# jacky121298/3DAL_PyTorch

Hardware: AMD Instinct MI355X
Metric: object-crops/sec through static+dynamic refinement heads (higher is better)
Workload: dtype f32; 1 GPU; StaticModelOneBoxEst forward+decode, 4096 crops x 1024 pts per GPU, fp32 (BASELINE.json configs[1]); items_per_gpu=4096, points_per_item=1024, sampler=device, parallelism=single GPU

## Files before the change

### 3dal_pytorch_amd/_hip.py

```python
import ctypes as C
import os

import numpy as np
import torch

_HERE = os.path.dirname(os.path.abspath(__file__))
LIB_PATH = os.path.join(_HERE, "lib3dal_hip.so")

OK, EINVAL, EWORKSPACE, EHIP = 0, -1, -2, -3
F32, BF16, F16, F16X3 = 0, 1, 2, 3
DTYPES = {"fp32": F32, "bf16": BF16, "fp16": F16, "f16x3": F16X3}
HEAD_INS_SEG, HEAD_STATIC_BOX_EST, HEAD_POINT_EMB, HEAD_BOX_EMB, HEAD_DYNAMIC_BOX_EST = range(5)
SAMPLER_DEVICE, SAMPLER_CHOICE = 0, 1
PHASE_SEG, PHASE_BOX, PHASE_ALL = 1, 2, 3

vp = C.c_void_p


class Layer(C.Structure):
    _fields_ = [("weight", vp), ("bias", vp), ("bn_weight", vp), ("bn_bias", vp), ("bn_mean", vp),
                ("bn_var", vp), ("c_in", C.c_int32), ("c_out", C.c_int32)]


class PackItem(C.Structure):
# ... 315 lines not shown
class AugmentBoxesArgs(C.Structure):
    _fields_ = [("B", C.c_int64), ("max_gt", C.c_int32), ("max_cand", C.c_int32), ("max_objs", C.c_int32), ("n_classes", C.c_int32),
                ("transform", C.c_int32), ("reserved", C.c_int32), ("gt_boxes", vp), ("gt_classes", vp), ("gt_counts", vp),
                ("cand_boxes", vp), ("cand_classes", vp), ("cand_counts", vp), ("accept", vp), ("xform", vp),
                ("range", C.c_float * 4), ("out", vp), ("out_count", vp), ("status", vp)]


_i, _i64, _u64, _sz = C.c_int, C.c_int64, C.c_uint64, C.c_size_t
SIGNATURES = {
    "dal3_version": (_i, []),
    "dal3_last_error": (C.c_char_p, []),
    "dal3_mean_size": (C.POINTER(C.c_float), []),
    "dal3_pack_weights": (_i, [_i, C.POINTER(Layer), _i, _i, vp, C.POINTER(_sz), vp]),
    "dal3_ins_seg_workspace_bytes": (_sz, [_i]),
    "dal3_ins_seg_plan_layout": (_i, [_i, C.POINTER(_sz), C.POINTER(_i)]),
    "dal3_ins_seg_forward": (_i, [vp, _i, _i, BCN, _i, _i, vp, vp, vp, vp, _sz, vp]),
    "dal3_ins_seg_encode": (_i, [vp, _i, _i, BCN, _i, _i, vp, vp]),
    "dal3_ins_seg_global_bias": (_i, [vp, _i, vp, _i, vp, vp]),
    "dal3_ins_seg_decode": (_i, [vp, _i, _i, BCN, _i, _i, vp, vp, vp, vp]),
    "dal3_gather_workspace_bytes": (_sz, [_i, _i]),
    "dal3_segment_counts": (_i, [vp, _i, _i, vp, vp]),
    "dal3_mask_compact_sample": (_i, [vp, BCN, _i, _i, _i, _i, _i, vp, _u64, _i64, vp, vp, vp, vp, _sz, vp]),
    "dal3_mask_compact_sample_step": (_i, [vp, BCN, _i, _i, _i, _i, _u64, vp, _i64, vp, vp, vp, vp, _sz, vp]),
    "dal3_point_head_workspace_bytes": (_sz, [_i]),
    "dal3_point_head_forward": (_i, [_i, vp, _i, BCN, _i, _i, vp, _i64, vp, _sz, vp]),
    "dal3_point_head_pool_workspace_bytes": (_sz, [_i, _i]),
    "dal3_point_head_screen_min_tiles": (_i, []),
    "dal3_point_head_screen_stride": (_i, []),
    "dal3_point_head_pool": (_i, [_i, vp, _i, BCN, _i, _i, vp, vp, vp, _sz, vp]),
    "dal3_dynamic_box_est_forward": (_i, [vp, vp, _i, vp, vp, _sz, vp]),
# ... 197 lines not shown
        if offsets.is_cuda:
            raise TypeError(f"{name} must be on the host (a list, an array or a CPU tensor): {sized_by} from it, and "
                            "reading a device tensor back would be the synchronisation this call avoids")
        offsets = offsets.numpy()
    off = np.ascontiguousarray(np.asarray(offsets, dtype=np.int64).reshape(-1))
    if off.size < 1:
        raise ValueError(f"{name} needs {count} + 1 entries")
    if off[0] < 0 or off[-1] > n or np.any(np.diff(off) < 0):
        raise ValueError(f"{name} must be non-decreasing within [0, {n}]")
    return off


STORAGE = {torch.float32: F32, torch.bfloat16: BF16, torch.float16: F16}
BCN_NO_SMALL_JOB_KERNELS, BCN_NO_WORKLIST, BCN_NO_LDS_SAMPLER = 1, 2, 4
BCN_NO_DEC_PLAN = 16
DISPATCH_FLAGS = 0


def bcn(t):
    assert t.dim() == 3 and t.dtype in STORAGE
    sb, sc, sn = t.stride()
    return BCN(ptr(t), sb, sc, sn, STORAGE[t.dtype], DISPATCH_FLAGS)


def layer_struct(conv, bn):
    w = conv.weight
    c_in, c_out = getattr(conv, "in_channels", w.shape[1]), getattr(conv, "out_channels", w.shape[0])
    if not w.is_contiguous() or w.dtype != torch.float32:
        raise RuntimeError("weights must be contiguous fp32")
    L = Layer(ptr(w), ptr(conv.bias), None, None, None, None, c_in, c_out)
# ... 45 lines not shown
```

### 3dal_pytorch_amd/csrc/dal3_api.hip

```cpp
#include <stdarg.h>
#include <stdio.h>
#include <string.h>

#include "dal3_block.h"
#include "dal3_kernels.h"
#include "dal3_lp.h"

static thread_local char g_err[512] = "";

static int fail(int code, const char* fmt, ...) {
    va_list ap;
    va_start(ap, fmt);
    vsnprintf(g_err, sizeof(g_err), fmt, ap);
    va_end(ap);
    return code;
}

#define HIP_TRY(expr)                                                                           \
    do {                                                                                        \
        hipError_t e_ = (expr);                                                                 \
        if (e_ != hipSuccess) return fail(DAL3_EHIP, "%s: %s", #expr, hipGetErrorString(e_)); \
    } while (0)
#define TRY(expr)               \
    do {                        \
// ... 456 lines not shown
        HIP_TRY(launch_pack_weight(L[3], PACK_ROWMAJOR, 0, 256, 0, 0, mut(w.w4row), s));
        HIP_TRY(launch_pack_weight_lp(L[3], DAL3_F16, 0, 0, 256, 16, 8, reinterpret_cast<uint16_t*>(mut(w.w4h)), s));
        HIP_TRY(launch_pack_head_screen(L[3], mut(w.scr_pq), reinterpret_cast<int32_t*>(mut(w.scr_flag)), s));
    }
    return pack_fc(L + 4, w.fc, s);
}

static BCN to_bcn(const dal3_bcn& t) { return BCN{t.data, t.stride_b, t.stride_c, t.stride_n, t.dtype, t.flags}; }

static int check_bcn(const dal3_bcn& t, const char* what) {
    if (!t.data) return fail(DAL3_EINVAL, "%s: null data pointer", what);
    if (t.stride_n <= 0 || t.stride_c <= 0) return fail(DAL3_EINVAL, "%s: strides must be positive", what);
    if (t.dtype != DAL3_F32 && t.dtype != DAL3_BF16 && t.dtype != DAL3_F16)
        return fail(DAL3_EINVAL, "%s: storage dtype %d is none of DAL3_F32 / DAL3_BF16 / DAL3_F16", what, t.dtype);
    if (t.dtype != DAL3_F32 && (reinterpret_cast<uintptr_t>(t.data) & 1)) return fail(DAL3_EINVAL, "%s: 16-bit data must be 2-byte aligned", what);
    if (t.flags & ~(DAL3_BCN_NO_SMALL_JOB_KERNELS | DAL3_BCN_NO_WORKLIST | DAL3_BCN_NO_LDS_SAMPLER | DAL3_BCN_NO_DEC_PLAN)) return fail(DAL3_EINVAL, "%s: unknown bits in flags (%d)", what, t.flags);
    return 0;
}

static int check_extent(int64_t B, int64_t N, const char* what) {
    if (B <= 0 || N <= 0) return fail(DAL3_EINVAL, "%s: B and N must be positive (B=%lld N=%lld)", what, (long long)B, (long long)N);
    if (B > DAL3_MAX_ITEMS) return fail(DAL3_EINVAL, "%s: B=%lld items exceed DAL3_MAX_ITEMS (%d)", what, (long long)B, DAL3_MAX_ITEMS);
    if (N > DAL3_MAX_POINTS_PER_ITEM)
        return fail(DAL3_EINVAL, "%s: N=%lld points per item exceed DAL3_MAX_POINTS_PER_ITEM (%d)", what, (long long)N, DAL3_MAX_POINTS_PER_ITEM);
    if (B * ((N + 31) / 32) > (int64_t)DAL3_MAX_TILES)
        return fail(DAL3_EINVAL, "%s: B=%lld x N=%lld is %lld 32-point tiles, more than DAL3_MAX_TILES (%d): split the batch", what,
                    (long long)B, (long long)N, (long long)(B * ((N + 31) / 32)), DAL3_MAX_TILES);
    return 0;
}

struct InsSegWs { float* g; float* gb; uint32_t* prune; uint32_t* plan_k; float* plan_gbc; int32_t* plan_nch; };
// ... 10 lines not shown
extern "C" size_t dal3_ins_seg_workspace_bytes(int B) {
    Carver c(nullptr, 0);
    carve_ins_seg(c, B);
    return c.off;
}

extern "C" int dal3_ins_seg_plan_layout(int B, size_t off[4], int* min_dead) {
    if (B <= 0 || !off) return fail(DAL3_EINVAL, "ins_seg_plan_layout: bad argument");
    char* const origin = reinterpret_cast<char*>(uintptr_t(4096));
    Carver c(origin, ~size_t(0));
    const InsSegWs w = carve_ins_seg(c, B);
    off[0] = reinterpret_cast<char*>(w.prune) - origin, off[1] = reinterpret_cast<char*>(w.plan_k) - origin;
    off[2] = reinterpret_cast<char*>(w.plan_gbc) - origin, off[3] = reinterpret_cast<char*>(w.plan_nch) - origin;
    if (min_dead) *min_dead = DAL3_DEC_MIN_DEAD;
    return 0;
}

static int check_dtype(int dtype) {
    if (dtype != DAL3_F32 && dtype != DAL3_BF16 && dtype != DAL3_F16 && dtype != DAL3_F16X3)
        return fail(DAL3_EINVAL, "unknown dtype %d", dtype);
    return 0;
}

static int ins_seg_run(const void* packed, int dtype, int c_in, const dal3_bcn& pts, int B, int N, float* logits,
                       uint8_t* mask, float* global_feat_out, const InsSegWs& ws, hipStream_t s) {
    TRY(check_dtype(dtype));
    if (!packed || !logits || !mask) return fail(DAL3_EINVAL, "ins_seg: null pointer");
    TRY(check_extent(B, N, "ins_seg"));
    if (c_in != 3 && c_in != 4) return fail(DAL3_EINVAL, "ins_seg: c_in must be 3 or 4");
    TRY(check_bcn(pts, "pts"));
// ... 2079 lines not shown
```

### 3dal_pytorch_amd/csrc/dal3_enc_screen.hip

```cpp
#include "dal3_device.h"
#include "dal3_kernels.h"
#include "dal3_lp.h"
#include "dal3_screen.h"

#ifndef SCR_CAP
#define SCR_CAP 1024
#endif
#define SCR_XLD 132
#define SCR_STAGE_LD 36
#ifndef SCR_DEPTH
#define SCR_DEPTH 2
#endif
#define SCR_XMAX_BITS 0x476A6000
#ifndef DAL3_SCR_A_STRIDE
#define DAL3_SCR_A_STRIDE 4
#endif
static_assert(DAL3_SCR_A_STRIDE >= 1, "pass A's stride over the wave-slots");

#ifdef DAL3_SCREEN_COUNT
__device__ unsigned long long g_scr_count[8];
extern "C" int dal3_debug_screen_counts(unsigned long long* out, int reset) {
    hipError_t e = hipMemcpyFromSymbol(out, HIP_SYMBOL(g_scr_count), sizeof(g_scr_count));
    if (e == hipSuccess && reset) {
        unsigned long long z[8] = {};
// ... 57 lines not shown
    for (int mt = 0; mt < 16; ++mt) {
#pragma unroll
        for (int j = 0; j < T; ++j) acc[mt & 1][j] = f32x16{};
#pragma unroll
        for (int i = 0; i < 4; ++i) {
            const f16x8_t a = __builtin_bit_cast(f16x8_t, r16.slot[i]);
            r16.slot[i] = r16.fetch();
#pragma unroll
            for (int j = 0; j < T; ++j) acc[mt & 1][j] = FP16::mfma(xh[j][i >> 1].k[i & 1], a, acc[mt & 1][j]);
        }
        if (mt > 0) fold(acc[(mt - 1) & 1], mt - 1);
    }
    fold(acc[1], 15);
}

template <int PASS, int T>
__global__ __launch_bounds__(64 * DAL3_WG_WAVES) void ins_seg_encode_screen_kernel(InsSegW w, BCN pts, int c_in, int n_pts,
                                                                                  int tiles_per_item, float* __restrict__ g,
                                                                                  uint32_t* __restrict__ prune) {
    const int lane = threadIdx.x & 63;
    const int wave = threadIdx.x >> 6;
    const int h = lane >> 5;
    const int64_t b = blockIdx.x / tiles_per_item;
    const int n0 = ((blockIdx.x % tiles_per_item) * DAL3_WG_WAVES + wave) * (PASS == 0 ? DAL3_SCR_A_STRIDE : 1) * (32 * T);
    __shared__ float s_b5[1024];
    __shared__ int s_max[1024];
    __shared__ f32x2 s_pq[1024];
    __shared__ float s_g[PASS == 1 ? 1024 : 1];
    __shared__ __attribute__((aligned(16))) float s_x[PASS == 1 ? DAL3_WG_WAVES * 32 * SCR_XLD : 4];
    __shared__ uint32_t s_list[PASS == 1 ? DAL3_WG_WAVES * T * SCR_CAP : 1];
    __shared__ __attribute__((aligned(16))) uint32_t s_stage[PASS == 1 ? DAL3_WG_WAVES * 64 * SCR_STAGE_LD : 4];
    __shared__ uint32_t s_u[PASS == 1 ? 512 : 1];
    __shared__ int s_xn[1];
    int* gi = reinterpret_cast<int*>(g + b * 1024);
    static_assert(22 * 1024 + 64 + DAL3_WG_WAVES * (32 * SCR_XLD * 4 + T * SCR_CAP * 4 + 64 * SCR_STAGE_LD * 4) <= 160 * 1024,
                  "pass B's LDS exceeds a CU's 160 KiB: lower SCR_CAP, DAL3_WG_WAVES or DAL3_ENC_T");
    static_assert(32 * 64 <= 64 * SCR_STAGE_LD, "a wave's stage holds the hit words of conv5's 32 blocks");
    if (PASS == 0 && *w.scr_flag != 0) return;
    for (int i = threadIdx.x; i < 1024; i += 64 * DAL3_WG_WAVES) {
        s_b5[i] = w.b5[i];
        s_max[i] = 0;
        s_pq[i] = reinterpret_cast<const f32x2*>(w.scr_pq)[i];
        if (PASS == 1) s_g[i] = __int_as_float(__hip_atomic_load(gi + i, __ATOMIC_RELAXED, __HIP_MEMORY_SCOPE_AGENT));
        if (PASS == 1 && i < 512) s_u[i] = 0;
    }
    if (threadIdx.x == 0) s_xn[0] = 0;
    __syncthreads();
    if (n0 < n_pts) {
        WRing<DAL3_PF> ring;
        ring.init(w.enc_stream, lane);
        f32x16 bias = tile_from_channels(w.b2, h);
        float in[T][2];
        load_points<2, T>(pts, b, n0, n_pts, c_in, in, lane);
        f32x16 x1[T][2], x2[T][2], x3[T][2], x4[T][4];
        first_layer<2, 2, T>(w.w1, w.b1, in, x1, lane);
        mlp_layer_ring<2, 2, T>(ring, w.b2, w.b3, bias, x1, x2, lane);
        if (PASS == 1 && prune) dec_prune_sweep<T>(w, x2, s_u, s_xn, lane);
        mlp_layer_ring<2, 2, T>(ring, w.b3, w.b4, bias, x2, x3, lane);
        mlp_layer_ring<2, 4, T>(ring, w.b4, w.b4, bias, x3, x4, lane);
        SCR_COUNT(0, 1);

        int xm = 0;
#pragma unroll
        for (int j = 0; j < T; ++j) {
#pragma unroll
            for (int kt = 0; kt < 4; ++kt) {
#pragma unroll
                for (int r = 0; r < 16; ++r) {
                    const int v = __float_as_int(x4[j][kt][r]);
                    xm = v > xm ? v : xm;
                }
            }
        }
        const bool dense = *w.scr_flag != 0 || __builtin_amdgcn_ballot_w64(xm > SCR_XMAX_BITS) != 0;
        if (dense) {
            SCR_COUNT(1, 1);
            if (PASS == 1) conv_max_layer<4, T>(ring, s_b5, x4, reinterpret_cast<float*>(s_max), 32, lane);
        } else {
            float x2max = 0.0f;
#pragma unroll
            for (int j = 0; j < T; ++j) {
                float ss = 0.0f;
#pragma unroll
                for (int kt = 0; kt < 4; ++kt) {
#pragma unroll
                    for (int r = 0; r < 16; ++r) ss = fmaf(x4[j][kt][r], x4[j][kt][r], ss);
                }
                ss += __shfl_xor(ss, 32);
                x2max = __builtin_fmaxf(x2max, ss);
            }
#pragma unroll
            for (int d = 16; d >= 1; d >>= 1) x2max = __builtin_fmaxf(x2max, __shfl_xor(x2max, d));
            const float X = sqrtf(x2max) * (1.0f + 0x1p-16f);

            ActTile<FP16> xh[T][4];
#pragma unroll
            for (int j = 0; j < T; ++j) {
#pragma unroll
                for (int kt = 0; kt < 4; ++kt) xh[j][kt] = pack_relu<FP16>(x4[j][kt]);
            }

            uint32_t* const list = s_list + (PASS == 1 ? wave * T * SCR_CAP : 0);
            uint32_t* const stage = s_stage + (PASS == 1 ? wave * 64 * SCR_STAGE_LD : 0);
            ScreenHits<T> hits;
            hits.init();

            auto block_const = [&](int mt) -> float {
                const int c = 32 * mt + (lane & 31);
                const f32x2 pq = s_pq[c];
                float E = fmaf(X, pq[0], pq[1]);
                E = fmaf(E, 0x1p-20f, E);
                if (PASS == 0) return E;
                const float G = s_g[c], bb = s_b5[c];
                if (bits_nonfinite(G)) return 3.0e38f;
                return (G - bb) - fmaf(__builtin_fabsf(G) + __builtin_fabsf(bb), 0x1p-22f, E);
            };
            static_assert(16 * T <= 32, "one hit bit per (tile, register) in a 32-bit word");
            float m = 0.0f;
            uint32_t hb = 0;
            auto ep_slice = [&](const f32x16 (&acc)[T], int i, float k) {
#pragma unroll
                for (int rr = 0; rr < 2; ++rr) {
#pragma unroll
                    for (int j = 0; j < T; ++j) {
                        const int r = 2 * i + rr;
                        if (PASS == 0)
                            m = (r == 0 && j == 0) ? acc[0][0] : __builtin_fmaxf(m, acc[j][r]);
                        else
                            hb = scr_push_hit(hb, acc[j][r], k);
                    }
                }
            };
            auto ep_finish = [&](int mt, float k) {
                const int c = 32 * mt + (lane & 31);
                if (PASS == 0) {
                    m = __builtin_fmaxf(m, __shfl_xor(m, 32));
                    const float y = m - fmaf(__builtin_fabsf(m), 0x1p-22f, k);
                    int bits = __float_as_int(y + s_b5[c]);
                    bits = bits > 0 ? bits : 0;
                    if (lane < 32 && bits > 0) atomicMax(&s_max[c], bits);
                } else {
                    hits.park_block(stage, mt, hb, lane);
                }
            };

            WRing<8> r16;
            r16.init(w.w5h, lane);
            auto mm = [&](f32x16 (&acc)[T], auto side) {
#pragma unroll
                for (int j = 0; j < T; ++j) acc[j] = f32x16{};
#pragma unroll
                for (int i = 0; i < 8; ++i) {
                    const f16x8_t a = __builtin_bit_cast(f16x8_t, r16.slot[i]);
                    r16.slot[i] = r16.fetch();
#pragma unroll
                    for (int j = 0; j < T; ++j) acc[j] = FP16::mfma(xh[j][i >> 1].k[i & 1], a, acc[j]);
                    DAL3_SCHED_FENCE();
                    side(i);
                    DAL3_SCHED_FENCE();
                }
            };
            f32x16 accA[T], accB[T];
            float kA = block_const(0), kB;
            mm(accA, NoSide());
            int mt = 1;
            for (; mt + 1 < 32; mt += 2) {
                kB = block_const(mt);
                mm(accB, [&](int i) { ep_slice(accA, i, kA); });
                ep_finish(mt - 1, kA);
                kA = block_const(mt + 1);
                mm(accA, [&](int i) { ep_slice(accB, i, kB); });
                ep_finish(mt, kB);
            }
            kB = block_const(mt);
            mm(accB, [&](int i) { ep_slice(accA, i, kA); });
            ep_finish(mt - 1, kA);
#pragma unroll
            for (int i = 0; i < 8; ++i) ep_slice(accB, i, kB);
            ep_finish(mt, kB);

            if (PASS == 1) {
                uint32_t cnt[T];
                const bool overflow = scr_build_lists<T, 32, SCR_CAP>(stage, list, hits, cnt, lane);
#pragma unroll
                for (int j = 0; j < T; ++j) SCR_COUNT(3, cnt[j]);
                if (overflow) {
                    SCR_COUNT(2, 1);
                    WRing<DAL3_PF> r32;
                    r32.init(w.enc_stream + ENC_W5 * 64, lane);
                    conv_max_layer<4, T>(r32, s_b5, x4, reinterpret_cast<float*>(s_max), 32, lane);
                } else {
                    float* const xw = s_x + wave * 32 * SCR_XLD;
#pragma unroll
                    for (int j = 0; j < T; ++j) {
                        __builtin_amdgcn_wave_barrier();
#pragma unroll
                        for (int kt = 0; kt < 4; ++kt) {
#pragma unroll
                            for (int q = 0; q < 4; ++q) {
                                f32x4 v;
                                v[0] = x4[j][kt][4 * q + 0];
                                v[1] = x4[j][kt][4 * q + 1];
                                v[2] = x4[j][kt][4 * q + 2];
                                v[3] = x4[j][kt][4 * q + 3];
                                *reinterpret_cast<f32x4*>(xw + (lane & 31) * SCR_XLD + 32 * kt + 8 * q + 4 * h) = v;
                            }
                        }
                        __builtin_amdgcn_wave_barrier();
                        SCR_COUNT(4, (cnt[j] + 63) / 64);
                        scr_recompute<32, 4, SCR_DEPTH, true>(
                            w.w5row, 128, list + j * SCR_CAP, cnt[j], xw, SCR_XLD, stage, lane, [](uint32_t, bool) { return 0.0f; },
                            [&](float a, int c, uint32_t, bool live) {
                                int bits = __float_as_int(a + s_b5[c]);
                                bits = bits > 0 ? bits : 0;
                                if (live && bits > 0) atomicMax(&s_max[c], bits);
                            });
                    }
                }
            }
        }
    }
    __syncthreads();
    for (int c = threadIdx.x; c < 1024; c += 64 * DAL3_WG_WAVES) {
        const int v = s_max[c];
        if (v > 0) atomicMax(gi + c, v);
    }
    if (PASS == 1 && prune) {
        uint32_t* pu = prune + b * 513;
        for (int c = threadIdx.x; c < 512; c += 64 * DAL3_WG_WAVES) {
            const uint32_t v = s_u[c];
            if (v > 0) atomicMax(pu + c, v);
        }
        if (threadIdx.x == 0 && s_xn[0] > 0) atomicMax(reinterpret_cast<int*>(pu + 512), s_xn[0]);
    }
}

hipError_t launch_ins_seg_encode_screen(const InsSegW& w, BCN pts, int c_in, int B, int N, float* g, hipStream_t s, uint32_t* prune) {
    constexpr int T = DAL3_ENC_T;
    const int tpi = (N + 32 * DAL3_WG_WAVES * T - 1) / (32 * DAL3_WG_WAVES * T);
    const int slots = (N + 32 * T - 1) / (32 * T);
    const int tpi_a = ((slots + DAL3_SCR_A_STRIDE - 1) / DAL3_SCR_A_STRIDE + DAL3_WG_WAVES - 1) / DAL3_WG_WAVES;
    const dim3 grid_a((unsigned)((int64_t)B * tpi_a)), grid((unsigned)((int64_t)B * tpi)), block(64 * DAL3_WG_WAVES);
    hipLaunchKernelGGL((ins_seg_encode_screen_kernel<0, T>), grid_a, block, 0, s, w, pts, c_in, N, tpi_a, g, nullptr);
    hipError_t e = hipGetLastError();
    if (e != hipSuccess) return e;
    hipLaunchKernelGGL((ins_seg_encode_screen_kernel<1, T>), grid, block, 0, s, w, pts, c_in, N, tpi, g, prune);
    return hipGetLastError();
}
```

### 3dal_pytorch_amd/csrc/dal3_kernels.h

```cpp
#pragma once
#include <hip/hip_runtime.h>
#include <stddef.h>
#include <stdint.h>

#include "../../include/dal3.h"
#include "dal3_device.h"
#include "dal3_fold.h"

#ifndef DAL3_ENC_T
#define DAL3_ENC_T 2
#endif
#ifndef DAL3_DEC_T
#define DAL3_DEC_T 1
#endif
#ifndef DAL3_HEAD_T
#define DAL3_HEAD_T 1
#endif

#ifndef DAL3_ENC_SCREEN
#define DAL3_ENC_SCREEN 1
#endif

#ifndef DAL3_WG_WAVES
#define DAL3_WG_WAVES 4
// ... 159 lines not shown
hipError_t launch_pack_weight_lp(const dal3_layer& L, int dtype, int kt_major, int col_off, int n_cols, int mt_n, int kt_n,
                                 uint16_t* out, hipStream_t s, int grp_blocks = 0, int64_t grp_a0 = 0, int64_t grp_a1 = 0,
                                 int64_t grp_stride = 0);

size_t ins_seg_packed_floats(int c_in);
InsSegW ins_seg_view(const float* base, int c_in);
size_t point_head_packed_floats(int head_kind);
PointHeadW point_head_view(const float* base, int head_kind);
size_t fc_head_packed_floats();
FcW fc_head_view(const float* base);
void point_head_dims(int head_kind, int* c_in, int* ks, int c[4], int* n_fc, int fc_in[3], int fc_out[3]);

hipError_t launch_ins_seg_encode(const InsSegW& w, BCN pts, int c_in, int B, int N, float* g, hipStream_t s, uint32_t* prune = nullptr);
hipError_t launch_ins_seg_encode_screen(const InsSegW& w, BCN pts, int c_in, int B, int N, float* g, hipStream_t s, uint32_t* prune);
bool dec_plan_route(int flags, int B, int N);
hipError_t launch_pack_dec_prune(const dal3_layer& L, float* dw1c, float* pq, uint32_t* ident, int32_t* flag, hipStream_t s);
hipError_t launch_dec_plan(const InsSegW& w, const float* gb, const uint32_t* prune, int B, uint32_t* plan_k, float* plan_gbc,
                           int32_t* plan_nch, hipStream_t s);
hipError_t launch_pack_enc_screen(const dal3_layer& L, float* pq, int32_t* flag, hipStream_t s);
hipError_t launch_pack_dec_sparse(const dal3_layer& L, const float* db2, float* dw2c, int32_t* flag, hipStream_t s);
hipError_t launch_pack_dec_queue(const dal3_layer& L, int c_in, const float* bias, float* wcopy, int32_t* flag, hipStream_t s);
hipError_t launch_ins_seg_decode(const InsSegW& w, BCN pts, int c_in, int B, int N, const float* gbias,
                                 float* logits, uint8_t* mask, hipStream_t s, DecPlan plan = DecPlan{nullptr, nullptr, nullptr});
size_t point_head_worklist_bytes(int B, int M);
hipError_t launch_point_head(int head_kind, const PointHeadW& w, BCN x, int c_in, int B, int M, float* feat,
                             const int32_t* distinct, hipStream_t s, void* worklist = nullptr, size_t worklist_bytes = 0);
#ifndef DAL3_HEAD_SCR_STRIDE
#define DAL3_HEAD_SCR_STRIDE 4
#endif
#ifndef DAL3_HEAD_SCREEN
// ... 303 lines not shown
```

### 3dal_pytorch_amd/csrc/dal3_pointmlp.hip

```cpp
#include <stdlib.h>

#include <type_traits>

#include "dal3_device.h"
#include "dal3_kernels.h"

#ifdef DAL3_STAMP
__device__ long long* g_stamps = nullptr;
extern "C" int dal3_debug_set_stamps(void* p) {
    return (int)hipMemcpyToSymbol(HIP_SYMBOL(g_stamps), &p, sizeof(p));
}
#define STAMP(k)                                                                                  \
    do {                                                                                          \
        __builtin_amdgcn_sched_barrier(0);                                                        \
        unsigned long long t_;                                                                    \
        asm volatile("s_memtime %0\n\ts_waitcnt lgkmcnt(0)" : "=s"(t_)::"memory");               \
        __builtin_amdgcn_sched_barrier(0);                                                        \
        if (lane == 0 && blockIdx.x < 2048) g_stamps[(blockIdx.x * DAL3_WG_WAVES + wave) * 16 + (k)] = t_; \
    } while (0)
#else
#define STAMP(k)
#endif

#ifndef DAL3_ENC_LDS_MAX
// ... 776 lines not shown
#endif
#ifndef DAL3_LAT_MAX_TILES_DEC
#define DAL3_LAT_MAX_TILES_DEC DAL3_LAT_MAX_TILES
#endif
#ifndef DAL3_LAT_MAX_TILES_HEAD
#define DAL3_LAT_MAX_TILES_HEAD DAL3_LAT_MAX_TILES
#endif
bool lat_use(int64_t tiles, int flags, int64_t max_tiles) { return !(flags & DAL3_BCN_NO_SMALL_JOB_KERNELS) && tiles <= max_tiles; }

bool dec_plan_route(int flags, int B, int N) {
    const int64_t tiles = (int64_t)B * ((N + 31) / 32);
    if (flags & DAL3_BCN_NO_DEC_PLAN) return false;
    if (!DAL3_ENC_SCREEN || !DAL3_DEC_SPARSE || DAL3_DEC_T != 1) return false;
    if (lat_use(tiles, flags, DAL3_LAT_MAX_TILES_ENC) || lat_use(tiles, flags, DAL3_LAT_MAX_TILES_DEC)) return false;
    return !(DAL3_ENC_T > 1 && (int64_t)B * N <= 1024 * 64);
}

hipError_t launch_ins_seg_encode(const InsSegW& w, BCN pts, int c_in, int B, int N, float* g, hipStream_t s, uint32_t* prune) {
    if (lat_use((int64_t)B * ((N + 31) / 32), pts.flags, DAL3_LAT_MAX_TILES_ENC)) return launch_ins_seg_encode_lat(w, pts, c_in, B, N, g, s);
    constexpr int T = DAL3_ENC_T;
    if (T > 1 && (int64_t)B * N <= 1024 * 64) {
        const int tpi1 = tiles_per_item(N, 1);
        hipLaunchKernelGGL(ins_seg_encode_kernel<1>, dim3((unsigned)((int64_t)B * tpi1)), dim3(64 * DAL3_WG_WAVES), 0, s, w, pts, c_in, N, tpi1, g);
        return hipGetLastError();
    }
    if (DAL3_ENC_SCREEN) return launch_ins_seg_encode_screen(w, pts, c_in, B, N, g, s, prune);
    const int tpi = tiles_per_item(N, T);
    hipLaunchKernelGGL(ins_seg_encode_kernel<T>, dim3((unsigned)((int64_t)B * tpi)), dim3(64 * DAL3_WG_WAVES), 0, s, w, pts, c_in, N, tpi, g);
    return hipGetLastError();
}
// ... 88 lines not shown
```

### include/dal3.h

```cpp
#ifndef DAL3_H
#define DAL3_H

#include <stddef.h>
#include <stdint.h>

#ifdef __cplusplus
extern "C" {
#endif

typedef void* dal3_stream;

#define DAL3_VERSION 170

enum {
    DAL3_OK = 0,
    DAL3_EINVAL = -1,
    DAL3_EWORKSPACE = -2,
    DAL3_EHIP = -3
};

#define DAL3_MAX_ITEMS 16777216
#define DAL3_MAX_POINTS_PER_ITEM 16777216
#define DAL3_MAX_TILES 2147483647

// ... 26 lines not shown

int dal3_version(void);
const char* dal3_last_error(void);
const float* dal3_mean_size(void);

int dal3_pack_weights(int head_kind, const dal3_layer* layers, int n_layers, int dtype,
                      void* packed_dev, size_t* bytes_inout, dal3_stream stream);

typedef struct {
    const float* data;
    int64_t stride_b, stride_c, stride_n;
    int32_t dtype;
    int32_t flags;
} dal3_bcn;

enum { DAL3_BCN_NO_SMALL_JOB_KERNELS = 1, DAL3_BCN_NO_WORKLIST = 2, DAL3_BCN_NO_LDS_SAMPLER = 4, DAL3_BCN_NO_DEC_PLAN = 16 };

size_t dal3_ins_seg_workspace_bytes(int B);
int dal3_ins_seg_plan_layout(int B, size_t off[4], int* min_dead);
int dal3_ins_seg_forward(const void* packed, int dtype, int c_in, dal3_bcn pts, int B, int N,
                         float* logits, uint8_t* mask, float* global_feat_out,
                         void* workspace, size_t workspace_bytes, dal3_stream stream);

int dal3_ins_seg_encode(const void* packed, int dtype, int c_in, dal3_bcn pts, int B, int N, float* global_feat,
                        dal3_stream stream);
int dal3_ins_seg_global_bias(const void* packed, int dtype, const float* global_feat, int B, float* gbias,
                             dal3_stream stream);
int dal3_ins_seg_decode(const void* packed, int dtype, int c_in, dal3_bcn pts, int B, int N, const float* gbias,
                        float* logits, uint8_t* mask, dal3_stream stream);

size_t dal3_gather_workspace_bytes(int B, int N);
int dal3_segment_counts(const uint8_t* mask, int B, int N, int32_t* counts, dal3_stream stream);
int dal3_mask_compact_sample(const uint8_t* mask, dal3_bcn pts, int B, int N, int C, int M,
                             int sampler, const int32_t* choice, uint64_t seed, int64_t item_offset,
// ... 1030 lines not shown
```

Before: 247,200 object-crops/s.

## Add resident single-launch screened encoder with one workgroup per item

Adds a resident encoder kernel that gives each item one workgroup, runs the screening pre-pass on its first slot and then the candidate pass over all slots, keeping conv5's running max in LDS. The two-launch screening path (pass A then pass B with separate grids) is refactored into shared helpers. The resident kernel is chosen when B is at least three times the CU count. The aim is to drop a kernel launch and the global round-trip of the per-item max between the passes. The cost is that each workgroup now loops serially over its item's slots, and the screening threshold comes from a partial first pass, which may let more candidates survive.

```diff
diff --git a/3dal_pytorch_amd/_hip.py b/3dal_pytorch_amd/_hip.py
--- a/3dal_pytorch_amd/_hip.py
+++ b/3dal_pytorch_amd/_hip.py
@@ -353,6 +353,7 @@
     "dal3_pack_weights": (_i, [_i, C.POINTER(Layer), _i, _i, vp, C.POINTER(_sz), vp]),
     "dal3_ins_seg_workspace_bytes": (_sz, [_i]),
     "dal3_ins_seg_plan_layout": (_i, [_i, C.POINTER(_sz), C.POINTER(_i)]),
+    "dal3_ins_seg_encoder_route": (_i, [_i, _i, _i]),
     "dal3_ins_seg_forward": (_i, [vp, _i, _i, BCN, _i, _i, vp, vp, vp, vp, _sz, vp]),
     "dal3_ins_seg_encode": (_i, [vp, _i, _i, BCN, _i, _i, vp, vp]),
     "dal3_ins_seg_global_bias": (_i, [vp, _i, vp, _i, vp, vp]),
@@ -580,6 +581,8 @@
 STORAGE = {torch.float32: F32, torch.bfloat16: BF16, torch.float16: F16}
 BCN_NO_SMALL_JOB_KERNELS, BCN_NO_WORKLIST, BCN_NO_LDS_SAMPLER = 1, 2, 4
 BCN_NO_DEC_PLAN = 16
+BCN_NO_ENC_RESIDENT = 32
+ENC_ROUTE_LATENCY, ENC_ROUTE_DENSE, ENC_ROUTE_TWO_LAUNCH, ENC_ROUTE_RESIDENT = 0, 1, 2, 3
 DISPATCH_FLAGS = 0
 
 
diff --git a/3dal_pytorch_amd/csrc/dal3_api.hip b/3dal_pytorch_amd/csrc/dal3_api.hip
--- a/3dal_pytorch_amd/csrc/dal3_api.hip
+++ b/3dal_pytorch_amd/csrc/dal3_api.hip
@@ -494,7 +494,7 @@
     if (t.dtype != DAL3_F32 && t.dtype != DAL3_BF16 && t.dtype != DAL3_F16)
         return fail(DAL3_EINVAL, "%s: storage dtype %d is none of DAL3_F32 / DAL3_BF16 / DAL3_F16", what, t.dtype);
     if (t.dtype != DAL3_F32 && (reinterpret_cast<uintptr_t>(t.data) & 1)) return fail(DAL3_EINVAL, "%s: 16-bit data must be 2-byte aligned", what);
-    if (t.flags & ~(DAL3_BCN_NO_SMALL_JOB_KERNELS | DAL3_BCN_NO_WORKLIST | DAL3_BCN_NO_LDS_SAMPLER | DAL3_BCN_NO_DEC_PLAN)) return fail(DAL3_EINVAL, "%s: unknown bits in flags (%d)", what, t.flags);
+    if (t.flags & ~(DAL3_BCN_NO_SMALL_JOB_KERNELS | DAL3_BCN_NO_WORKLIST | DAL3_BCN_NO_LDS_SAMPLER | DAL3_BCN_NO_DEC_PLAN | DAL3_BCN_NO_ENC_RESIDENT)) return fail(DAL3_EINVAL, "%s: unknown bits in flags (%d)", what, t.flags);
     return 0;
 }
 
@@ -535,6 +535,13 @@
     off[2] = reinterpret_cast<char*>(w.plan_gbc) - origin, off[3] = reinterpret_cast<char*>(w.plan_nch) - origin;
     if (min_dead) *min_dead = DAL3_DEC_MIN_DEAD;
     return 0;
+}
+
+extern "C" int dal3_ins_seg_encoder_route(int B, int N, int flags) {
+    TRY(check_extent(B, N, "ins_seg_encoder_route"));
+    if (flags & ~(DAL3_BCN_NO_SMALL_JOB_KERNELS | DAL3_BCN_NO_WORKLIST | DAL3_BCN_NO_LDS_SAMPLER | DAL3_BCN_NO_DEC_PLAN | DAL3_BCN_NO_ENC_RESIDENT))
+        return fail(DAL3_EINVAL, "ins_seg_encoder_route: unknown bits in flags (%d)", flags);
+    return enc_route(flags, B, N);
 }
 
 static int check_dtype(int dtype) {
diff --git a/3dal_pytorch_amd/csrc/dal3_enc_screen.hip b/3dal_pytorch_amd/csrc/dal3_enc_screen.hip
--- a/3dal_pytorch_amd/csrc/dal3_enc_screen.hip
+++ b/3dal_pytorch_amd/csrc/dal3_enc_screen.hip
@@ -1,3 +1,4 @@
+#include <cstddef>
 #include "dal3_device.h"
 #include "dal3_kernels.h"
 #include "dal3_lp.h"
@@ -95,233 +96,303 @@
     fold(acc[1], 15);
 }
 
+template <bool CAND, int T>
+struct EncScreenLds {
+    float b5[1024];
+    int max[1024];
+    f32x2 pq[1024];
+    float g[CAND ? 1024 : 1];
+    float x[CAND ? DAL3_WG_WAVES * 32 * SCR_XLD : 4];
+    uint32_t list[CAND ? DAL3_WG_WAVES * T * SCR_CAP : 1];
+    uint32_t stage[CAND ? DAL3_WG_WAVES * 64 * SCR_STAGE_LD : 4];
+    uint32_t u[CAND ? 512 : 1];
+    int xn[1];
+};
+using EncScreenLdsB = EncScreenLds<true, DAL3_ENC_T>;
+static_assert(offsetof(EncScreenLdsB, x) % 16 == 0 && offsetof(EncScreenLdsB, stage) % 16 == 0,
+              "x and stage are read and written 16 bytes at a time (the struct itself is placed on 16 bytes)");
+static_assert(22 * 1024 + 64 + DAL3_WG_WAVES * (32 * SCR_XLD * 4 + DAL3_ENC_T * SCR_CAP * 4 + 64 * SCR_STAGE_LD * 4) <= 160 * 1024 &&
+                  sizeof(EncScreenLds<true, DAL3_ENC_T>) <= 22 * 1024 + 64 + DAL3_WG_WAVES * (32 * SCR_XLD * 4 + DAL3_ENC_T * SCR_CAP * 4 + 64 * SCR_STAGE_LD * 4),
+              "pass B's and the resident kernel's LDS exceeds a CU's 160 KiB: lower SCR_CAP, DAL3_WG_WAVES or DAL3_ENC_T");
+static_assert(32 * 64 <= 64 * SCR_STAGE_LD, "a wave's stage holds the hit words of conv5's 32 blocks");
+
+template <int PASS, bool RISING, int T, class Lds>
+__device__ __forceinline__ void scr_conv5_sweep(const InsSegW& w, const ActTile<FP16> (&xh)[T][4], float X, Lds& L, uint32_t* stage,
+                                                ScreenHits<T>& hits, int lane) {
+    auto block_const = [&](int mt) -> float {
+        const int c = 32 * mt + (lane & 31);
+        const f32x2 pq = L.pq[c];
+        float E = fmaf(X, pq[0], pq[1]);
+        E = fmaf(E, 0x1p-20f, E);
+        if (PASS == 0) return E;
+        float G = L.g[c];
+        const float bb = L.b5[c];
+        if (RISING) {
+            const int own = L.max[c], row = __float_as_int(G);
+            G = __int_as_float(own > row ? own : row);
+        }
+        if (bits_nonfinite(G)) return 3.0e38f;
+        return (G - bb) - fmaf(__builtin_fabsf(G) + __builtin_fabsf(bb), 0x1p-22f, E);
+    };
+    static_assert(16 * T <= 32, "one hit bit per (tile, register) in a 32-bit word");
+    float m = 0.0f;
+    uint32_t hb = 0;
+    auto ep_slice = [&](const f32x16 (&acc)[T], int i, float k) {
+#pragma unroll
+        for (int rr = 0; rr < 2; ++rr) {
+#pragma unroll
+            for (int j = 0; j < T; ++j) {
+                const int r = 2 * i + rr;
+                if (PASS == 0)
+                    m = (r == 0 && j == 0) ? acc[0][0] : __builtin_fmaxf(m, acc[j][r]);
+                else
+                    hb = scr_push_hit(hb, acc[j][r], k);
+            }
+        }
+    };
+    auto ep_finish = [&](int mt, float k) {
+        const int c = 32 * mt + (lane & 31);
+        if (PASS == 0) {
+            m = __builtin_fmaxf(m, __shfl_xor(m, 32));
+            const float y = m - fmaf(__builtin_fabsf(m), 0x1p-22f, k);
+            int bits = __float_as_int(y + L.b5[c]);
+            bits = bits > 0 ? bits : 0;
+            if (lane < 32 && bits > 0) atomicMax(&L.max[c], bits);
+        } else {
+            hits.park_block(stage, mt, hb, lane);
+        }
+    };
+
+    WRing<8> r16;
+    r16.init(w.w5h, lane);
+    auto mm = [&](f32x16 (&acc)[T], auto side) {
+#pragma unroll
+        for (int j = 0; j < T; ++j) acc[j] = f32x16{};
+#pragma unroll
+        for (int i = 0; i < 8; ++i) {
+            const f16x8_t a = __builtin_bit_cast(f16x8_t, r16.slot[i]);
+            r16.slot[i] = r16.fetch();
+#pragma unroll
+            for (int j = 0; j < T; ++j) acc[j] = FP16::mfma(xh[j][i >> 1].k[i & 1], a, acc[j]);
+            DAL3_SCHED_FENCE();
+            side(i);
+            DAL3_SCHED_FENCE();
+        }
+    };
+    f32x16 accA[T], accB[T];
+    float kA = block_const(0), kB;
+    mm(accA, NoSide());
+    int mt = 1;
+    for (; mt + 1 < 32; mt += 2) {
+        kB = block_const(mt);
+        mm(accB, [&](int i) { ep_slice(accA, i, kA); });
+        ep_finish(mt - 1, kA);
+        kA = block_const(mt + 1);
+        mm(accA, [&](int i) { ep_slice(accB, i, kB); });
+        ep_finish(mt, kB);
+    }
+    kB = block_const(mt);
+    mm(accB, [&](int i) { ep_slice(accA, i, kA); });
+    ep_finish(mt - 1, kA);
+#pragma unroll
+    for (int i = 0; i < 8; ++i) ep_slice(accB, i, kB);
+    ep_finish(mt, kB);
+}
+
+template <int MODE, int T, class Lds>
+__device__ __forceinline__ void enc_screen_slot(const InsSegW& w, BCN pts, int c_in, int n_pts, int64_t b, int n0, bool with_prune,
+                                                bool first, Lds& L, int lane, int wave) {
+    const int h = lane >> 5;
+    const bool active = n0 < n_pts;
+    f32x16 x4[T][4];
+    WRing<DAL3_PF> ring;
+    bool dense = false;
+    if (active) {
+        ring.init(w.enc_stream, lane);
+        f32x16 bias = tile_from_channels(w.b2, h);
+        float in[T][2];
+        load_points<2, T>(pts, b, n0, n_pts, c_in, in, lane);
+        f32x16 x1[T][2], x2[T][2], x3[T][2];
+        first_layer<2, 2, T>(w.w1, w.b1, in, x1, lane);
+        mlp_layer_ring<2, 2, T>(ring, w.b2, w.b3, bias, x1, x2, lane);
+        if (MODE != 0 && with_prune) dec_prune_sweep<T>(w, x2, L.u, L.xn, lane);
+        mlp_layer_ring<2, 2, T>(ring, w.b3, w.b4, bias, x2, x3, lane);
+        mlp_layer_ring<2, 4, T>(ring, w.b4, w.b4, bias, x3, x4, lane);
+        SCR_COUNT(0, 1);
+
+        int xm = 0;
+#pragma unroll
+        for (int j = 0; j < T; ++j) {
+#pragma unroll
+            for (int kt = 0; kt < 4; ++kt) {
+#pragma unroll
+                for (int r = 0; r < 16; ++r) {
+                    const int v = __float_as_int(x4[j][kt][r]);
+                    xm = v > xm ? v : xm;
+                }
+            }
+        }
+        dense = *w.scr_flag != 0 || __builtin_amdgcn_ballot_w64(xm > SCR_XMAX_BITS) != 0;
+        if (dense) {
+            SCR_COUNT(1, 1);
+            if (MODE == 1) conv_max_layer<4, T>(ring, L.b5, x4, reinterpret_cast<float*>(L.max), 32, lane);
+        }
+    }
+    const bool screened = active && !dense;
+    float X = 0.0f;
+    ActTile<FP16> xh[T][4];
+    if (screened) {
+        float x2max = 0.0f;
+#pragma unroll
+        for (int j = 0; j < T; ++j) {
+            float ss = 0.0f;
+#pragma unroll
+            for (int kt = 0; kt < 4; ++kt) {
+#pragma unroll
+                for (int r = 0; r < 16; ++r) ss = fmaf(x4[j][kt][r], x4[j][kt][r], ss);
+            }
+            ss += __shfl_xor(ss, 32);
+            x2max = __builtin_fmaxf(x2max, ss);
+        }
+#pragma unroll
+        for (int d = 16; d >= 1; d >>= 1) x2max = __builtin_fmaxf(x2max, __shfl_xor(x2max, d));
+        X = sqrtf(x2max) * (1.0f + 0x1p-16f);
+#pragma unroll
+        for (int j = 0; j < T; ++j) {
+#pragma unroll
+            for (int kt = 0; kt < 4; ++kt) xh[j][kt] = pack_relu<FP16>(x4[j][kt]);
+        }
+    }
+    uint32_t* const list = L.list + (MODE != 0 ? wave * T * SCR_CAP : 0);
+    uint32_t* const stage = L.stage + (MODE != 0 ? wave * 64 * SCR_STAGE_LD : 0);
+    ScreenHits<T> hits;
+    hits.init();
+    if (MODE == 2) {
+        if (first) {
+            if (screened) scr_conv5_sweep<0, false, T>(w, xh, X, L, stage, hits, lane);
+            __syncthreads();
+        }
+        if (active && dense) {
+            WRing<DAL3_PF> r32;
+            r32.init(w.enc_stream + ENC_W5 * 64, lane);
+            conv_max_layer<4, T>(r32, L.b5, x4, reinterpret_cast<float*>(L.max), 32, lane);
+        }
+    }
+    if (screened) {
+        scr_conv5_sweep<(MODE == 0 ? 0 : 1), MODE == 2, T>(w, xh, X, L, stage, hits, lane);
+        if (MODE != 0) {
+            uint32_t cnt[T];
+            const bool overflow = scr_build_lists<T, 32, SCR_CAP>(stage, list, hits, cnt, lane);
+#pragma unroll
+            for (int j = 0; j < T; ++j) SCR_COUNT(3, cnt[j]);
+            if (overflow) {
+                SCR_COUNT(2, 1);
+                WRing<DAL3_PF> r32;
+                r32.init(w.enc_stream + ENC_W5 * 64, lane);
+                conv_max_layer<4, T>(r32, L.b5, x4, reinterpret_cast<float*>(L.max), 32, lane);
+            } else {
+                float* const xw = L.x + wave * 32 * SCR_XLD;
+#pragma unroll
+                for (int j = 0; j < T; ++j) {
+                    __builtin_amdgcn_wave_barrier();
+#pragma unroll
+                    for (int kt = 0; kt < 4; ++kt) {
+#pragma unroll
+                        for (int q = 0; q < 4; ++q) {
+                            f32x4 v;
+                            v[0] = x4[j][kt][4 * q + 0];
+                            v[1] = x4[j][kt][4 * q + 1];
+                            v[2] = x4[j][kt][4 * q + 2];
+                            v[3] = x4[j][kt][4 * q + 3];
+                            *reinterpret_cast<f32x4*>(xw + (lane & 31) * SCR_XLD + 32 * kt + 8 * q + 4 * h) = v;
+                        }
+                    }
+                    __builtin_amdgcn_wave_barrier();
+                    SCR_COUNT(4, (cnt[j] + 63) / 64);
+                    scr_recompute<32, 4, SCR_DEPTH, true>(
+                        w.w5row, 128, list + j * SCR_CAP, cnt[j], xw, SCR_XLD, stage, lane, [](uint32_t, bool) { return 0.0f; },
+                        [&](float a, int c, uint32_t, bool live) {
+                            int bits = __float_as_int(a + L.b5[c]);
+                            bits = bits > 0 ? bits : 0;
+                            if (live && bits > 0) atomicMax(&L.max[c], bits);
+                        });
+                }
+            }
+        }
+    }
+}
+
+template <bool CAND, int T>
+__device__ __forceinline__ void enc_screen_tables(const InsSegW& w, EncScreenLds<CAND, T>& L, int* gi) {
+    for (int i = threadIdx.x; i < 1024; i += 64 * DAL3_WG_WAVES) {
+        L.b5[i] = w.b5[i];
+        L.max[i] = 0;
+        L.pq[i] = reinterpret_cast<const f32x2*>(w.scr_pq)[i];
+        if (CAND) L.g[i] = __int_as_float(__hip_atomic_load(gi + i, __ATOMIC_RELAXED, __HIP_MEMORY_SCOPE_AGENT));
+        if (CAND && i < 512) L.u[i] = 0;
+    }
+    if (threadIdx.x == 0) L.xn[0] = 0;
+    __syncthreads();
+}
+template <bool CAND, int T>
+__device__ __forceinline__ void enc_screen_flush(EncScreenLds<CAND, T>& L, int* gi, uint32_t* pu) {
+    __syncthreads();
+    for (int c = threadIdx.x; c < 1024; c += 64 * DAL3_WG_WAVES) {
+        const int v = L.max[c];
+        if (v > 0) atomicMax(gi + c, v);
+    }
+    if (CAND && pu) {
+        for (int c = threadIdx.x; c < 512; c += 64 * DAL3_WG_WAVES) {
+            const uint32_t v = L.u[c];
+            if (v > 0) atomicMax(pu + c, v);
+        }
+        if (threadIdx.x == 0 && L.xn[0] > 0) atomicMax(reinterpret_cast<int*>(pu + 512), L.xn[0]);
+    }
+}
+
 template <int PASS, int T>
 __global__ __launch_bounds__(64 * DAL3_WG_WAVES) void ins_seg_encode_screen_kernel(InsSegW w, BCN pts, int c_in, int n_pts,
                                                                                   int tiles_per_item, float* __restrict__ g,
                                                                                   uint32_t* __restrict__ prune) {
     const int lane = threadIdx.x & 63;
     const int wave = threadIdx.x >> 6;
-    const int h = lane >> 5;
     const int64_t b = blockIdx.x / tiles_per_item;
     const int n0 = ((blockIdx.x % tiles_per_item) * DAL3_WG_WAVES + wave) * (PASS == 0 ? DAL3_SCR_A_STRIDE : 1) * (32 * T);
-    __shared__ float s_b5[1024];
-    __shared__ int s_max[1024];
-    __shared__ f32x2 s_pq[1024];
-    __shared__ float s_g[PASS == 1 ? 1024 : 1];
-    __shared__ __attribute__((aligned(16))) float s_x[PASS == 1 ? DAL3_WG_WAVES * 32 * SCR_XLD : 4];
-    __shared__ uint32_t s_list[PASS == 1 ? DAL3_WG_WAVES * T * SCR_CAP : 1];
-    __shared__ __attribute__((aligned(16))) uint32_t s_stage[PASS == 1 ? DAL3_WG_WAVES * 64 * SCR_STAGE_LD : 4];
-    __shared__ uint32_t s_u[PASS == 1 ? 512 : 1];
-    __shared__ int s_xn[1];
+    __shared__ __attribute__((aligned(16))) EncScreenLds<PASS == 1, T> L;
     int* gi = reinterpret_cast<int*>(g + b * 1024);
-    static_assert(22 * 1024 + 64 + DAL3_WG_WAVES * (32 * SCR_XLD * 4 + T * SCR_CAP * 4 + 64 * SCR_STAGE_LD * 4) <= 160 * 1024,
-                  "pass B's LDS exceeds a CU's 160 KiB: lower SCR_CAP, DAL3_WG_WAVES or DAL3_ENC_T");
-    static_assert(32 * 64 <= 64 * SCR_STAGE_LD, "a wave's stage holds the hit words of conv5's 32 blocks");
     if (PASS == 0 && *w.scr_flag != 0) return;
-    for (int i = threadIdx.x; i < 1024; i += 64 * DAL3_WG_WAVES) {
-        s_b5[i] = w.b5[i];
-        s_max[i] = 0;
-        s_pq[i] = reinterpret_cast<const f32x2*>(w.scr_pq)[i];
-        if (PASS == 1) s_g[i] = __int_as_float(__hip_atomic_load(gi + i, __ATOMIC_RELAXED, __HIP_MEMORY_SCOPE_AGENT));
-        if (PASS == 1 && i < 512) s_u[i] = 0;
-    }
-    if (threadIdx.x == 0) s_xn[0] = 0;
-    __syncthreads();
-    if (n0 < n_pts) {
-        WRing<DAL3_PF> ring;
-        ring.init(w.enc_stream, lane);
-        f32x16 bias = tile_from_channels(w.b2, h);
-        float in[T][2];
-        load_points<2, T>(pts, b, n0, n_pts, c_in, in, lane);
-        f32x16 x1[T][2], x2[T][2], x3[T][2], x4[T][4];
-        first_layer<2, 2, T>(w.w1, w.b1, in, x1, lane);
-        mlp_layer_ring<2, 2, T>(ring, w.b2, w.b3, bias, x1, x2, lane);
-        if (PASS == 1 && prune) dec_prune_sweep<T>(w, x2, s_u, s_xn, lane);
-        mlp_layer_ring<2, 2, T>(ring, w.b3, w.b4, bias, x2, x3, lane);
-        mlp_layer_ring<2, 4, T>(ring, w.b4, w.b4, bias, x3, x4, lane);
-        SCR_COUNT(0, 1);
-
-        int xm = 0;
-#pragma unroll
-        for (int j = 0; j < T; ++j) {
-#pragma unroll
-            for (int kt = 0; kt < 4; ++kt) {
-#pragma unroll
-                for (int r = 0; r < 16; ++r) {
-                    const int v = __float_as_int(x4[j][kt][r]);
-                    xm = v > xm ? v : xm;
-                }
-            }
-        }
-        const bool dense = *w.scr_flag != 0 || __builtin_amdgcn_ballot_w64(xm > SCR_XMAX_BITS) != 0;
-        if (dense) {
-            SCR_COUNT(1, 1);
-            if (PASS == 1) conv_max_layer<4, T>(ring, s_b5, x4, reinterpret_cast<float*>(s_max), 32, lane);
-        } else {
-            float x2max = 0.0f;
-#pragma unroll
-            for (int j = 0; j < T; ++j) {
-                float ss = 0.0f;
-#pragma unroll
-                for (int kt = 0; kt < 4; ++kt) {
-#pragma unroll
-                    for (int r = 0; r < 16; ++r) ss = fmaf(x4[j][kt][r], x4[j][kt][r], ss);
-                }
-                ss += __shfl_xor(ss, 32);
-                x2max = __builtin_fmaxf(x2max, ss);
-            }
-#pragma unroll
-            for (int d = 16; d >= 1; d >>= 1) x2max = __builtin_fmaxf(x2max, __shfl_xor(x2max, d));
-            const float X = sqrtf(x2max) * (1.0f + 0x1p-16f);
-
-            ActTile<FP16> xh[T][4];
-#pragma unroll
-            for (int j = 0; j < T; ++j) {
-#pragma unroll
-                for (int kt = 0; kt < 4; ++kt) xh[j][kt] = pack_relu<FP16>(x4[j][kt]);
-            }
-
-            uint32_t* const list = s_list + (PASS == 1 ? wave * T * SCR_CAP : 0);
-            uint32_t* const stage = s_stage + (PASS == 1 ? wave * 64 * SCR_STAGE_LD : 0);
-            ScreenHits<T> hits;
-            hits.init();
-
-            auto block_const = [&](int mt) -> float {
-                const int c = 32 * mt + (lane & 31);
-                const f32x2 pq = s_pq[c];
-                float E = fmaf(X, pq[0], pq[1]);
-                E = fmaf(E, 0x1p-20f, E);
-                if (PASS == 0) return E;
-                const float G = s_g[c], bb = s_b5[c];
-                if (bits_nonfinite(G)) return 3.0e38f;
-                return (G - bb) - fmaf(__builtin_fabsf(G) + __builtin_fabsf(bb), 0x1p-22f, E);
-            };
-            static_assert(16 * T <= 32, "one hit bit per (tile, register) in a 32-bit word");
-            float m = 0.0f;
-            uint32_t hb = 0;
-            auto ep_slice = [&](const f32x16 (&acc)[T], int i, float k) {
-#pragma unroll
-                for (int rr = 0; rr < 2; ++rr) {
-#pragma unroll
-                    for (int j = 0; j < T; ++j) {
-                        const int r = 2 * i + rr;
-                        if (PASS == 0)
-                            m = (r == 0 && j == 0) ? acc[0][0] : __builtin_fmaxf(m, acc[j][r]);
-                        else
-                            hb = scr_push_hit(hb, acc[j][r], k);
-                    }
-                }
-            };
-            auto ep_finish = [&](int mt, float k) {
-                const int c = 32 * mt + (lane & 31);
-                if (PASS == 0) {
-                    m = __builtin_fmaxf(m, __shfl_xor(m, 32));
-                    const float y = m - fmaf(__builtin_fabsf(m), 0x1p-22f, k);
-                    int bits = __float_as_int(y + s_b5[c]);
-                    bits = bits > 0 ? bits : 0;
-                    if (lane < 32 && bits > 0) atomicMax(&s_max[c], bits);
-                } else {
-                    hits.park_block(stage, mt, hb, lane);
-                }
-            };
-
-            WRing<8> r16;
-            r16.init(w.w5h, lane);
-            auto mm = [&](f32x16 (&acc)[T], auto side) {
-#pragma unroll
-                for (int j = 0; j < T; ++j) acc[j] = f32x16{};
-#pragma unroll
-                for (int i = 0; i < 8; ++i) {
-                    const f16x8_t a = __builtin_bit_cast(f16x8_t, r16.slot[i]);
-                    r16.slot[i] = r16.fetch();
-#pragma unroll
-                    for (int j = 0; j < T; ++j) acc[j] = FP16::mfma(xh[j][i >> 1].k[i & 1], a, acc[j]);
-                    DAL3_SCHED_FENCE();
-                    side(i);
-                    DAL3_SCHED_FENCE();
-                }
-            };
-            f32x16 accA[T], accB[T];
-            float kA = block_const(0), kB;
-            mm(accA, NoSide());
-            int mt = 1;
-            for (; mt + 1 < 32; mt += 2) {
-                kB = block_const(mt);
-                mm(accB, [&](int i) { ep_slice(accA, i, kA); });
-                ep_finish(mt - 1, kA);
-                kA = block_const(mt + 1);
-                mm(accA, [&](int i) { ep_slice(accB, i, kB); });
-                ep_finish(mt, kB);
-            }
-            kB = block_const(mt);
-            mm(accB, [&](int i) { ep_slice(accA, i, kA); });
-            ep_finish(mt - 1, kA);
-#pragma unroll
-            for (int i = 0; i < 8; ++i) ep_slice(accB, i, kB);
-            ep_finish(mt, kB);
-
-            if (PASS == 1) {
-                uint32_t cnt[T];
-                const bool overflow = scr_build_lists<T, 32, SCR_CAP>(stage, list, hits, cnt, lane);
-#pragma unroll
-                for (int j = 0; j < T; ++j) SCR_COUNT(3, cnt[j]);
-                if (overflow) {
-                    SCR_COUNT(2, 1);
-                    WRing<DAL3_PF> r32;
-                    r32.init(w.enc_stream + ENC_W5 * 64, lane);
-                    conv_max_layer<4, T>(r32, s_b5, x4, reinterpret_cast<float*>(s_max), 32, lane);
-                } else {
-                    float* const xw = s_x + wave * 32 * SCR_XLD;
-#pragma unroll
-                    for (int j = 0; j < T; ++j) {
-                        __builtin_amdgcn_wave_barrier();
-#pragma unroll
-                        for (int kt = 0; kt < 4; ++kt) {
-#pragma unroll
-                            for (int q = 0; q < 4; ++q) {
-                                f32x4 v;
-                                v[0] = x4[j][kt][4 * q + 0];
-                                v[1] = x4[j][kt][4 * q + 1];
-                                v[2] = x4[j][kt][4 * q + 2];
-                                v[3] = x4[j][kt][4 * q + 3];
-                                *reinterpret_cast<f32x4*>(xw + (lane & 31) * SCR_XLD + 32 * kt + 8 * q + 4 * h) = v;
-                            }
-                        }
-                        __builtin_amdgcn_wave_barrier();
-                        SCR_COUNT(4, (cnt[j] + 63) / 64);
-                        scr_recompute<32, 4, SCR_DEPTH, true>(
-                            w.w5row, 128, list + j * SCR_CAP, cnt[j], xw, SCR_XLD, stage, lane, [](uint32_t, bool) { return 0.0f; },
-                            [&](float a, int c, uint32_t, bool live) {
-                                int bits = __float_as_int(a + s_b5[c]);
-                                bits = bits > 0 ? bits : 0;
-                                if (live && bits > 0) atomicMax(&s_max[c], bits);
-                            });
-                    }
-                }
-            }
-        }
-    }
-    __syncthreads();
-    for (int c = threadIdx.x; c < 1024; c += 64 * DAL3_WG_WAVES) {
-        const int v = s_max[c];
-        if (v > 0) atomicMax(gi + c, v);
-    }
-    if (PASS == 1 && prune) {
-        uint32_t* pu = prune + b * 513;
-        for (int c = threadIdx.x; c < 512; c += 64 * DAL3_WG_WAVES) {
-            const uint32_t v = s_u[c];
-            if (v > 0) atomicMax(pu + c, v);
-        }
-        if (threadIdx.x == 0 && s_xn[0] > 0) atomicMax(reinterpret_cast<int*>(pu + 512), s_xn[0]);
-    }
+    enc_screen_tables(w, L, gi);
+    enc_screen_slot<PASS, T>(w, pts, c_in, n_pts, b, n0, prune != nullptr, false, L, lane, wave);
+    enc_screen_flush(L, gi, PASS == 1 && prune ? prune + b * 513 : nullptr);
+}
+
+template <int T>
+__global__ __launch_bounds__(64 * DAL3_WG_WAVES) void ins_seg_encode_resident_kernel(InsSegW w, BCN pts, int c_in, int n_pts,
+                                                                                    float* __restrict__ g, uint32_t* __restrict__ prune) {
+    const int lane = threadIdx.x & 63;
+    const int wave = threadIdx.x >> 6;
+    const int64_t b = blockIdx.x;
+    __shared__ __attribute__((aligned(16))) EncScreenLds<true, T> L;
+    int* gi = reinterpret_cast<int*>(g + b * 1024);
+    enc_screen_tables(w, L, gi);
+    const int slots = (n_pts + 32 * T - 1) / (32 * T);
+    const int R = (slots + DAL3_WG_WAVES - 1) / DAL3_WG_WAVES;
+    for (int r = 0; r < R; ++r)
+        enc_screen_slot<2, T>(w, pts, c_in, n_pts, b, (r + R * wave) * (32 * T), prune != nullptr, r == 0, L, lane, wave);
+    enc_screen_flush(L, gi, prune ? prune + b * 513 : nullptr);
 }
 
 hipError_t launch_ins_seg_encode_screen(const InsSegW& w, BCN pts, int c_in, int B, int N, float* g, hipStream_t s, uint32_t* prune) {
     constexpr int T = DAL3_ENC_T;
+    const dim3 block(64 * DAL3_WG_WAVES);
+    if (enc_resident_route(pts.flags, B, N)) {
+        hipLaunchKernelGGL((ins_seg_encode_resident_kernel<T>), dim3((unsigned)B), block, 0, s, w, pts, c_in, N, g, prune);
+        return hipGetLastError();
+    }
     const int tpi = (N + 32 * DAL3_WG_WAVES * T - 1) / (32 * DAL3_WG_WAVES * T);
     const int slots = (N + 32 * T - 1) / (32 * T);
     const int tpi_a = ((slots + DAL3_SCR_A_STRIDE - 1) / DAL3_SCR_A_STRIDE + DAL3_WG_WAVES - 1) / DAL3_WG_WAVES;
-    const dim3 grid_a((unsigned)((int64_t)B * tpi_a)), grid((unsigned)((int64_t)B * tpi)), block(64 * DAL3_WG_WAVES);
+    const dim3 grid_a((unsigned)((int64_t)B * tpi_a)), grid((unsigned)((int64_t)B * tpi));
     hipLaunchKernelGGL((ins_seg_encode_screen_kernel<0, T>), grid_a, block, 0, s, w, pts, c_in, N, tpi_a, g, nullptr);
     hipError_t e = hipGetLastError();
     if (e != hipSuccess) return e;
diff --git a/3dal_pytorch_amd/csrc/dal3_kernels.h b/3dal_pytorch_amd/csrc/dal3_kernels.h
--- a/3dal_pytorch_amd/csrc/dal3_kernels.h
+++ b/3dal_pytorch_amd/csrc/dal3_kernels.h
@@ -197,6 +197,8 @@
 hipError_t launch_ins_seg_encode(const InsSegW& w, BCN pts, int c_in, int B, int N, float* g, hipStream_t s, uint32_t* prune = nullptr);
 hipError_t launch_ins_seg_encode_screen(const InsSegW& w, BCN pts, int c_in, int B, int N, float* g, hipStream_t s, uint32_t* prune);
 bool dec_plan_route(int flags, int B, int N);
+int enc_route(int flags, int B, int N);
+bool enc_resident_route(int flags, int B, int N);
 hipError_t launch_pack_dec_prune(const dal3_layer& L, float* dw1c, float* pq, uint32_t* ident, int32_t* flag, hipStream_t s);
 hipError_t launch_dec_plan(const InsSegW& w, const float* gb, const uint32_t* prune, int B, uint32_t* plan_k, float* plan_gbc,
                            int32_t* plan_nch, hipStream_t s);
diff --git a/3dal_pytorch_amd/csrc/dal3_pointmlp.hip b/3dal_pytorch_amd/csrc/dal3_pointmlp.hip
--- a/3dal_pytorch_amd/csrc/dal3_pointmlp.hip
+++ b/3dal_pytorch_amd/csrc/dal3_pointmlp.hip
@@ -814,6 +814,30 @@
     if (!DAL3_ENC_SCREEN || !DAL3_DEC_SPARSE || DAL3_DEC_T != 1) return false;
     if (lat_use(tiles, flags, DAL3_LAT_MAX_TILES_ENC) || lat_use(tiles, flags, DAL3_LAT_MAX_TILES_DEC)) return false;
     return !(DAL3_ENC_T > 1 && (int64_t)B * N <= 1024 * 64);
+}
+
+#ifndef DAL3_ENC_RES_MIN_PER_CU
+#define DAL3_ENC_RES_MIN_PER_CU 3
+#endif
+static int enc_cu_count() {
+    static int n = 0;
+    if (n == 0) {
+        int dev = 0, v = 0;
+        if (hipGetDevice(&dev) != hipSuccess || hipDeviceGetAttribute(&v, hipDeviceAttributeMultiprocessorCount, dev) != hipSuccess || v <= 0)
+            v = 256;
+        n = v;
+    }
+    return n;
+}
+bool enc_resident_route(int flags, int B, int N) {
+    (void)N;
+    return !(flags & DAL3_BCN_NO_ENC_RESIDENT) && (int64_t)B >= (int64_t)DAL3_ENC_RES_MIN_PER_CU * enc_cu_count();
+}
+int enc_route(int flags, int B, int N) {
+    if (lat_use((int64_t)B * ((N + 31) / 32), flags, DAL3_LAT_MAX_TILES_ENC)) return DAL3_ENC_ROUTE_LATENCY;
+    if (DAL3_ENC_T > 1 && (int64_t)B * N <= 1024 * 64) return DAL3_ENC_ROUTE_DENSE;
+    if (!DAL3_ENC_SCREEN) return DAL3_ENC_ROUTE_DENSE;
+    return enc_resident_route(flags, B, N) ? DAL3_ENC_ROUTE_RESIDENT : DAL3_ENC_ROUTE_TWO_LAUNCH;
 }
 
 hipError_t launch_ins_seg_encode(const InsSegW& w, BCN pts, int c_in, int B, int N, float* g, hipStream_t s, uint32_t* prune) {
diff --git a/include/dal3.h b/include/dal3.h
--- a/include/dal3.h
+++ b/include/dal3.h
@@ -64,10 +64,13 @@
     int32_t flags;
 } dal3_bcn;
 
-enum { DAL3_BCN_NO_SMALL_JOB_KERNELS = 1, DAL3_BCN_NO_WORKLIST = 2, DAL3_BCN_NO_LDS_SAMPLER = 4, DAL3_BCN_NO_DEC_PLAN = 16 };
+enum { DAL3_BCN_NO_SMALL_JOB_KERNELS = 1, DAL3_BCN_NO_WORKLIST = 2, DAL3_BCN_NO_LDS_SAMPLER = 4, DAL3_BCN_NO_DEC_PLAN = 16,
+       DAL3_BCN_NO_ENC_RESIDENT = 32 };
 
 size_t dal3_ins_seg_workspace_bytes(int B);
 int dal3_ins_seg_plan_layout(int B, size_t off[4], int* min_dead);
+enum { DAL3_ENC_ROUTE_LATENCY = 0, DAL3_ENC_ROUTE_DENSE = 1, DAL3_ENC_ROUTE_TWO_LAUNCH = 2, DAL3_ENC_ROUTE_RESIDENT = 3 };
+int dal3_ins_seg_encoder_route(int B, int N, int flags);
 int dal3_ins_seg_forward(const void* packed, int dtype, int c_in, dal3_bcn pts, int B, int N,
                          float* logits, uint8_t* mask, float* global_feat_out,
                          void* workspace, size_t workspace_bytes, dal3_stream stream);
```

After: 263,200 object-crops/s, median of 6. 1.06x the previous value.
